# ArchieGertsman/spark-sched-sim

Hardware: AMD Instinct MI355X
Metric: env-steps/sec at 4096 batched envs (TPC-H, 10 exec) (higher is better)
Workload: dtype int64+f64

## Files before the change

### include/sss.h

```cpp
#ifndef SSS_H
#define SSS_H
#include <stddef.h>
#include <stdint.h>

#ifdef __cplusplus
extern "C" {
#endif

typedef struct sss_handle sss_handle;

typedef struct sss_cfg {
  int32_t num_executors;
  int32_t job_arrival_cap;
  int32_t max_jobs;
  int32_t reserved;
  double job_arrival_rate;
  double moving_delay;
  double warmup_delay;
  double beta;
} sss_cfg;

typedef struct sss_dims {
  int32_t num_envs, num_executors, job_cap, stage_stride;
  int32_t node_cap;
// ... 24 lines not shown
  SSS_E_STALLED = 5,
  SSS_E_NO_DURATION = 6,
  SSS_E_INVARIANT = 7,
  SSS_E_NEED_RESET = 8,
  SSS_E_NO_LIMIT = 9,
  SSS_E_CAPACITY = 10
};

int sss_query_dims(const sss_cfg* cfg, const void* pack, size_t pack_bytes, int num_envs, sss_dims* out);

int sss_create(const sss_cfg* cfg, const void* pack, size_t pack_bytes, int num_envs, int device, sss_handle** out);

int sss_bind_buffers(sss_handle* h, const sss_buffers* buffers);

int sss_reset(sss_handle* h, const uint64_t* seeds_dev, const double* time_limits_dev, const uint8_t* mask_dev, void* stream);

#define SSS_SKIP_ENV (-2147483647 - 1)
int sss_step(sss_handle* h, const int32_t* stage_idx_dev, const int32_t* num_exec_dev, int auto_reset, uint64_t seed_stride, void* stream);

int sss_step_bounded(sss_handle* h, const int32_t* stage_idx_dev, const int32_t* num_exec_dev, int auto_reset, uint64_t seed_stride, int max_events,
                     uint8_t* ready_dev, void* stream);

int sss_policy(sss_handle* h, int policy, int param, int32_t* stage_idx_dev, int32_t* num_exec_dev, void* stream);

int sss_rollout(sss_handle* h, int policy, int param, int n_steps, int auto_reset, uint64_t seed_stride, void* stream);

typedef struct sss_decima_graph {
  const uint8_t* active_dev;
  const int64_t* node_off_dev;
  const int64_t* job_off_dev;
  const int64_t* edge_off_dev;
  float num_tasks_scale;
  float work_scale;
  float* x_dev;
  int64_t* node_obs_dev;
  int64_t* node_loc_dev;
  int64_t* node_job_dev;
  int64_t* sched_rank_dev;
  int32_t* gen_dev;
  uint32_t* node_recv_dev;
  uint8_t* stage_mask_dev;
  int64_t* src_dev;
  int64_t* dst_dev;
  int64_t* edge_obs_dev;
  uint32_t* edge_layers_dev;
  int64_t* job_obs_dev;
// ... 383 lines not shown
```

### spark_sched_sim_amd/binding.py

```python
from __future__ import annotations

import ctypes as C
import os.path as osp

CSRC = osp.join(osp.dirname(osp.abspath(__file__)), "csrc")
LIB_NAME = "libsss_hip.so"


class SssCfg(C.Structure):
    _fields_ = [("num_executors", C.c_int32), ("job_arrival_cap", C.c_int32), ("max_jobs", C.c_int32),
                ("reserved", C.c_int32), ("job_arrival_rate", C.c_double), ("moving_delay", C.c_double),
                ("warmup_delay", C.c_double), ("beta", C.c_double)]


class SssDims(C.Structure):
    _fields_ = [("num_envs", C.c_int32), ("num_executors", C.c_int32), ("job_cap", C.c_int32),
                ("stage_stride", C.c_int32), ("node_cap", C.c_int32), ("edge_cap", C.c_int32),
                ("obs_i32", C.c_int32), ("obs_f64", C.c_int32), ("state_bytes", C.c_int64),
                ("env_stride", C.c_int64), ("off_t_arrival", C.c_int64), ("off_t_completed", C.c_int64),
                ("off_jobs", C.c_int64), ("off_active", C.c_int64), ("off_dur_ring", C.c_int64),
                ("job_rec_bytes", C.c_int32), ("hdr_bytes", C.c_int32)]


class SssBuffers(C.Structure):
# ... 137 lines not shown
    _fields_ = [("env_ids_dev", C.c_void_p), ("n", C.c_int32), ("width", C.c_int32), ("height", C.c_int32), ("pad_", C.c_int32), ("rgb_dev", C.c_void_p)]


JOB_STATS_COLUMNS = ("num_jobs", "total_job_time", "avg_job_duration", "avg_num_jobs", "avg_completed_job_duration", "num_completed_jobs", "num_active_jobs",
                     "wall_time")
JOB_STATS_MAX_Q = 16

REWARD_WINDOW_CHUNK = 64


def reward_window_scratch(T: int, B: int) -> int:
    return ((T + REWARD_WINDOW_CHUNK - 1) // REWARD_WINDOW_CHUNK + 1) * B + 1


class SssArenaArray(C.Structure):
    _fields_ = [("src_dev", C.c_void_p), ("dst_dev", C.c_void_p), ("elem_bytes", C.c_int32), ("per_row", C.c_int32), ("kind", C.c_int32), ("shift", C.c_int32)]


class SssArenaArgs(C.Structure):
    _fields_ = [("n_arrays", C.c_int32), ("n_obs", C.c_int32), ("totals_dev", C.c_void_p), ("cursor_dev", C.c_void_p), ("capacity", C.c_int64 * 4),
                ("rows_hint", C.c_int64), ("arrays", SssArenaArray * 24)]


EXPORTS = ["sss_query_dims", "sss_create", "sss_bind_buffers", "sss_reset", "sss_step", "sss_step_bounded", "sss_policy", "sss_rollout",
           "sss_decima_graph_build", "sss_decima_layer_lists", "sss_prefix_rows", "sss_decima_policy", "sss_decima_sample", "sss_gnn_launch",
           "sss_linear_wgrad_scratch", "sss_linear_wgrad", "sss_mlp_supported", "sss_mlp_recompute_supported", "sss_mlp_split_supported", "sss_mlp_forward", "sss_mlp_backward", "sss_mlp_wgrad_scratch", "sss_mlp_backward_wgrad", "sss_mlp_wgrad_finish", "sss_collect_step", "sss_gnn_encode", "sss_rows_op", "sss_rows_concat", "sss_segment_categorical", "sss_bit_lists", "sss_arena_append", "sss_discounted_returns", "sss_sequence_baselines", "sss_reward_window_update", "sss_differential_returns", "sss_bind_timeline", "sss_timeline_render", "sss_decima_argmax", "sss_decima_policy_argmax", "sss_job_stats", "sss_last_error", "sss_destroy", "sss_abi_sizeof"]
POLICY_IDS = {"fair": 0, "fifo": 1, "hash": 2, "wfair": 3, "sjfcp": 4}
WFAIR_ALPHA_RANGE = (-4, 4)
ABI_STRUCTS = {"sss_cfg": SssCfg, "sss_dims": SssDims, "sss_buffers": SssBuffers, "sss_decima_graph": SssDecimaGraph, "sss_decima_lists": SssDecimaLists,
               "sss_bit_list_args": SssBitListArgs, "sss_gnn_args": SssGnnArgs, "sss_decima_policy_args": SssDecimaPolicyArgs,
               "sss_decima_sample_args": SssDecimaSampleArgs, "sss_gnn_encode_args": SssGnnEncodeArgs, "sss_collect_args": SssCollectArgs,
               "sss_mlp_args": SssMlpArgs, "sss_arena_array": SssArenaArray, "sss_arena_args": SssArenaArgs, "sss_returns_args": SssReturnsArgs,
               "sss_baseline_args": SssBaselineArgs, "sss_rows_args": SssRowsArgs, "sss_concat_part": SssConcatPart, "sss_concat_args": SssConcatArgs, "sss_segcat_args": SssSegcatArgs}
ABI_TAGGED_STRUCTS = {"sss_reward_window_args": SssRewardWindowArgs, "sss_diffret_args": SssDiffretArgs}
ABI_PLAIN_STRUCTS = {"sss_timeline": SssTimeline, "sss_timeline_render_args": SssTimelineRenderArgs}


def load_library(path: str | None = None) -> C.CDLL:
    path = path or osp.join(CSRC, LIB_NAME)
    if not osp.exists(path):
        raise RuntimeError(
            f"{path} not found: the HIP extension has not been built "
            "(run `python -c 'import __graft_entry__ as g; g.build()'` or spark_sched_sim_amd/build.py). "
            "There is no CPU fallback.")
    return C.CDLL(path)


class Binding:
    def __init__(self, lib: C.CDLL | None = None):
        self.lib = lib if lib is not None else load_library()
        L = self.lib
        L.sss_query_dims.argtypes = [C.POINTER(SssCfg), C.c_void_p, C.c_size_t, C.c_int, C.POINTER(SssDims)]
        L.sss_create.argtypes = [C.POINTER(SssCfg), C.c_void_p, C.c_size_t, C.c_int, C.c_int, C.POINTER(C.c_void_p)]
        L.sss_bind_buffers.argtypes = [C.c_void_p, C.POINTER(SssBuffers)]
        L.sss_reset.argtypes = [C.c_void_p, C.c_void_p, C.c_void_p, C.c_void_p, C.c_void_p]
        L.sss_step.argtypes = [C.c_void_p, C.c_void_p, C.c_void_p, C.c_int, C.c_uint64, C.c_void_p]
        L.sss_step_bounded.argtypes = [C.c_void_p, C.c_void_p, C.c_void_p, C.c_int, C.c_uint64, C.c_int, C.c_void_p, C.c_void_p]
        L.sss_policy.argtypes = [C.c_void_p, C.c_int, C.c_int, C.c_void_p, C.c_void_p, C.c_void_p]
        L.sss_rollout.argtypes = [C.c_void_p, C.c_int, C.c_int, C.c_int, C.c_int, C.c_uint64, C.c_void_p]
        L.sss_decima_graph_build.argtypes = [C.c_void_p, C.POINTER(SssDecimaGraph), C.c_void_p]
        L.sss_decima_layer_lists.argtypes = [C.c_int, C.POINTER(SssDecimaLists), C.c_void_p]
        L.sss_prefix_rows.argtypes = [C.c_void_p, C.c_int64, C.c_int64, C.c_void_p, C.c_int, C.c_int, C.c_void_p, C.c_void_p, C.c_void_p, C.c_void_p]
        L.sss_decima_policy.argtypes = [C.c_void_p, C.POINTER(SssDecimaPolicyArgs), C.c_void_p]
        L.sss_decima_sample.argtypes = [C.c_int, C.c_int, C.POINTER(SssDecimaSampleArgs), C.c_void_p]
        L.sss_gnn_launch.argtypes = [C.c_int, C.POINTER(SssGnnArgs), C.c_void_p]
        L.sss_linear_wgrad_scratch.argtypes = [C.c_int, C.c_int]
        L.sss_linear_wgrad_scratch.restype = C.c_int64
        L.sss_linear_wgrad.argtypes = [C.c_void_p, C.c_int64, C.c_void_p, C.c_int64, C.c_int64, C.c_int, C.c_int, C.c_void_p, C.c_void_p, C.c_void_p, C.c_void_p]
        L.sss_gnn_encode.argtypes = [C.POINTER(SssGnnEncodeArgs), C.c_void_p]
        L.sss_collect_step.argtypes = [C.POINTER(SssCollectArgs), C.c_int, C.c_void_p]
        L.sss_mlp_supported.argtypes = [C.c_int] * 5
        L.sss_mlp_recompute_supported.argtypes = [C.c_int]
        L.sss_mlp_split_supported.argtypes = [C.c_int]
        L.sss_mlp_forward.argtypes = [C.POINTER(SssMlpArgs), C.c_void_p]
        L.sss_mlp_backward.argtypes = [C.POINTER(SssMlpArgs), C.c_void_p]
        L.sss_mlp_wgrad_scratch.argtypes = [C.c_int]
        L.sss_mlp_wgrad_scratch.restype = C.c_int64
        L.sss_mlp_backward_wgrad.argtypes = [C.POINTER(SssMlpArgs), C.c_void_p, C.c_void_p]
        L.sss_mlp_wgrad_finish.argtypes = [C.c_int] + [C.c_void_p] * 8
        L.sss_discounted_returns.argtypes = [C.POINTER(SssReturnsArgs), C.c_void_p]
# ... 46 lines not shown
```

### spark_sched_sim_amd/csrc/sss_hip_sim.hip

```cpp
#include <hip/hip_runtime.h>

#include "sss_sim.h"
#include "sss_narrow.h"

#ifdef SSS_TIMELINE
#define SSS_LAUNCHER(name) sss_narrow_tl_launch_##name
#define SSS_TL_DISPATCH(call)
#else
#define SSS_LAUNCHER(name) sss_narrow_launch_##name
#define SSS_TL_DISPATCH(call) \
  if (a.tl.t) return sss_narrow_tl_launch_##call
int sss_narrow_hot_bytes() { return (int)sizeof(SssHot); }
int sss_narrow_static_lds_bytes() { return SSS_STATIC_LDS_BYTES; }
#endif

int SSS_LAUNCHER(reset)(const SssKernelArgs& a, int num_envs, const uint64_t* seeds, const double* tl, const uint8_t* mask, void* stream) {
  SSS_TL_DISPATCH(reset(a, num_envs, seeds, tl, mask, stream));
  hipLaunchKernelGGL(SSS_KNAME(sss_reset_kernel), dim3(num_envs), dim3(64), (size_t)a.P.pool_bytes, (hipStream_t)stream, a, seeds, tl, mask);
  return (int)hipGetLastError();
}
int SSS_LAUNCHER(step_bounded)(const SssKernelArgs& a, int num_envs, const int32_t* stage_idx, const int32_t* num_exec, int auto_reset, uint64_t seed_stride,
                                   int budget, uint8_t* ready, void* stream) {
  SSS_TL_DISPATCH(step_bounded(a, num_envs, stage_idx, num_exec, auto_reset, seed_stride, budget, ready, stream));
  hipLaunchKernelGGL(SSS_KNAME(sss_step_bounded_kernel), dim3(num_envs), dim3(64), (size_t)a.P.pool_bytes, (hipStream_t)stream, a, stage_idx, num_exec, auto_reset, seed_stride,
                     budget, ready);
  return (int)hipGetLastError();
}
int SSS_LAUNCHER(step)(const SssKernelArgs& a, int num_envs, const int32_t* stage_idx, const int32_t* num_exec, int auto_reset, uint64_t seed_stride,
                           void* stream) {
  SSS_TL_DISPATCH(step(a, num_envs, stage_idx, num_exec, auto_reset, seed_stride, stream));
  hipLaunchKernelGGL(SSS_KNAME(sss_step_kernel), dim3(num_envs), dim3(64), (size_t)a.P.pool_bytes, (hipStream_t)stream, a, stage_idx, num_exec, auto_reset, seed_stride);
  return (int)hipGetLastError();
}
#ifndef SSS_TIMELINE
int SSS_LAUNCHER(policy)(const SssKernelArgs& a, int num_envs, int policy, int param, int32_t* stage_idx, int32_t* num_exec, void* stream) {
  hipLaunchKernelGGL(SSS_KNAME(sss_policy_kernel), dim3(num_envs), dim3(64), (size_t)a.P.pool_bytes, (hipStream_t)stream, a, policy, param, stage_idx, num_exec);
  return (int)hipGetLastError();
}
#endif
int SSS_LAUNCHER(rollout)(const SssKernelArgs& a, int num_envs, int policy, int param, int n_steps, int auto_reset, uint64_t seed_stride, void* stream) {
  SSS_TL_DISPATCH(rollout(a, num_envs, policy, param, n_steps, auto_reset, seed_stride, stream));
  if (policy >= SSS_POLICY_WFAIR)
    hipLaunchKernelGGL(SSS_KNAME(sss_rollout_heur_kernel), dim3(num_envs), dim3(64), (size_t)a.P.pool_bytes, (hipStream_t)stream, a, policy, param, n_steps, auto_reset, seed_stride);
  else
    hipLaunchKernelGGL(SSS_KNAME(sss_rollout_kernel), dim3(num_envs), dim3(64), (size_t)a.P.pool_bytes, (hipStream_t)stream, a, policy, param, n_steps, auto_reset, seed_stride);
  return (int)hipGetLastError();
}

#if defined(SSS_EVPROF3) && !defined(SSS_TIMELINE)
extern "C" int sss_debug_prof(unsigned long long* out64) {
  if (hipMemcpyFromSymbol(out64, HIP_SYMBOL(g_prof3), sizeof(unsigned long long) * 96) != hipSuccess) return -1;
  static const unsigned long long zeros[96] = {0};
  return hipMemcpyToSymbol(HIP_SYMBOL(g_prof3), zeros, sizeof(zeros)) == hipSuccess ? 0 : -1;
}
extern "C" int sss_debug_prof_min(unsigned long long min_step_ticks) {
  return hipMemcpyToSymbol(HIP_SYMBOL(g_prof3_min), &min_step_ticks, sizeof(min_step_ticks)) == hipSuccess ? 0 : -1;
}
#endif
```

### spark_sched_sim_amd/csrc/sss_hip_wide.hip

```cpp
#define SSS_WIDE 1
#include <hip/hip_runtime.h>

#include "sss_sim.h"
#include "sss_wide.h"

#ifdef SSS_TIMELINE
#define SSS_LAUNCHER(name) sss_wide_tl_launch_##name
#define SSS_TL_DISPATCH(call)
#else
#define SSS_LAUNCHER(name) sss_wide_launch_##name
#define SSS_TL_DISPATCH(call) \
  if (a.tl.t) return sss_wide_tl_launch_##call
int sss_wide_hot_bytes() { return (int)sizeof(SssHot); }
int sss_wide_static_lds_bytes() { return SSS_STATIC_LDS_BYTES; }
#endif

int SSS_LAUNCHER(reset)(const SssKernelArgs& a, int num_envs, const uint64_t* seeds, const double* tl, const uint8_t* mask, void* stream) {
  SSS_TL_DISPATCH(reset(a, num_envs, seeds, tl, mask, stream));
  hipLaunchKernelGGL(SSS_KNAME(sss_reset_kernel), dim3(num_envs), dim3(64), (size_t)a.P.pool_bytes, (hipStream_t)stream, a, seeds, tl, mask);
  return (int)hipGetLastError();
}
int SSS_LAUNCHER(step_bounded)(const SssKernelArgs& a, int num_envs, const int32_t* stage_idx, const int32_t* num_exec, int auto_reset, uint64_t seed_stride,
                                 int budget, uint8_t* ready, void* stream) {
  SSS_TL_DISPATCH(step_bounded(a, num_envs, stage_idx, num_exec, auto_reset, seed_stride, budget, ready, stream));
  hipLaunchKernelGGL(SSS_KNAME(sss_step_bounded_kernel), dim3(num_envs), dim3(64), (size_t)a.P.pool_bytes, (hipStream_t)stream, a, stage_idx, num_exec, auto_reset,
                     seed_stride, budget, ready);
  return (int)hipGetLastError();
}
int SSS_LAUNCHER(step)(const SssKernelArgs& a, int num_envs, const int32_t* stage_idx, const int32_t* num_exec, int auto_reset, uint64_t seed_stride,
                         void* stream) {
  SSS_TL_DISPATCH(step(a, num_envs, stage_idx, num_exec, auto_reset, seed_stride, stream));
  hipLaunchKernelGGL(SSS_KNAME(sss_step_kernel), dim3(num_envs), dim3(64), (size_t)a.P.pool_bytes, (hipStream_t)stream, a, stage_idx, num_exec, auto_reset, seed_stride);
  return (int)hipGetLastError();
}
#ifndef SSS_TIMELINE
int SSS_LAUNCHER(policy)(const SssKernelArgs& a, int num_envs, int policy, int param, int32_t* stage_idx, int32_t* num_exec, void* stream) {
  hipLaunchKernelGGL(SSS_KNAME(sss_policy_kernel), dim3(num_envs), dim3(64), (size_t)a.P.pool_bytes, (hipStream_t)stream, a, policy, param, stage_idx, num_exec);
  return (int)hipGetLastError();
}
#endif
int SSS_LAUNCHER(rollout)(const SssKernelArgs& a, int num_envs, int policy, int param, int n_steps, int auto_reset, uint64_t seed_stride, void* stream) {
  SSS_TL_DISPATCH(rollout(a, num_envs, policy, param, n_steps, auto_reset, seed_stride, stream));
  if (policy >= SSS_POLICY_WFAIR)
    hipLaunchKernelGGL(SSS_KNAME(sss_rollout_heur_kernel), dim3(num_envs), dim3(64), (size_t)a.P.pool_bytes, (hipStream_t)stream, a, policy, param, n_steps, auto_reset, seed_stride);
  else
    hipLaunchKernelGGL(SSS_KNAME(sss_rollout_kernel), dim3(num_envs), dim3(64), (size_t)a.P.pool_bytes, (hipStream_t)stream, a, policy, param, n_steps, auto_reset, seed_stride);
  return (int)hipGetLastError();
}

#if defined(SSS_EVPROF3) && !defined(SSS_TIMELINE)
extern "C" int sss_debug_prof_wide(unsigned long long* out64) {
  if (hipMemcpyFromSymbol(out64, HIP_SYMBOL(g_prof3), sizeof(unsigned long long) * 96) != hipSuccess) return -1;
  static const unsigned long long zeros[96] = {0};
  return hipMemcpyToSymbol(HIP_SYMBOL(g_prof3), zeros, sizeof(zeros)) == hipSuccess ? 0 : -1;
}
extern "C" int sss_debug_prof_min_wide(unsigned long long min_step_ticks) {
  return hipMemcpyToSymbol(HIP_SYMBOL(g_prof3_min), &min_step_ticks, sizeof(min_step_ticks)) == hipSuccess ? 0 : -1;
}
#endif
```

### spark_sched_sim_amd/csrc/sss_host.h

```cpp
#pragma once
#include <math.h>
#include <stdio.h>
#include <stdlib.h>
#include <string.h>

#include <string>
#include <vector>

#include "../../include/sss.h"
#include "sss_layout.h"
#include "sss_train.h"
#include "sss_rows.h"
#include "sss_narrow.h"
#include "sss_wide.h"
#include "sss_timeline.h"
#include "sss_jobstats.h"

static bool sss_is_wide(int num_executors) { return num_executors > 64; }
static int sss_hot_bytes(int num_executors) { return sss_is_wide(num_executors) ? sss_wide_hot_bytes() : sss_narrow_hot_bytes(); }

static thread_local std::string g_sss_err;
static int sss_fail(int code, const std::string& msg) {
  g_sss_err = msg;
  return code;
// ... 460 lines not shown
  if (max_events < 1) return sss_fail(-35, "sss_step_bounded: max_events must be at least 1");
  BeDeviceGuard guard(h->device);
  const SssKernelArgs ka = sss_args(h);
  if (int rc = sss_is_wide(h->L.E) ? sss_wide_launch_step_bounded(ka, h->L.num_envs, stage_idx_dev, num_exec_dev, auto_reset, seed_stride, max_events, ready_dev, stream)
                                   : be_launch_step_bounded(ka, h->L.num_envs, stage_idx_dev, num_exec_dev, auto_reset, seed_stride, max_events, ready_dev, stream))
    return sss_fail(-30, std::string("step launch failed: ") + be_error(rc));
  return 0;
}

static int sss_check_policy(int policy, int param) {
  if (policy < 0 || policy > 4) return sss_fail(-23, "unknown policy");
  if (policy == 3 && (param < -4 || param > 4)) return sss_fail(-23, "weighted fair: alpha (param) must be in [-4, 4], got " + std::to_string(param));
  return 0;
}

extern "C" int sss_policy(sss_handle* h, int policy, int param, int32_t* stage_idx_dev, int32_t* num_exec_dev, void* stream) {
  if (!h || !stage_idx_dev || !num_exec_dev) return sss_fail(-1, "NULL argument");
  if (!h->bound) return sss_fail(-22, "sss_bind_buffers has not been called");
  BeDeviceGuard guard(h->device);
  if (int rc = sss_check_policy(policy, param)) return rc;
  const SssKernelArgs ka = sss_args(h);
  if (int rc = sss_is_wide(h->L.E) ? sss_wide_launch_policy(ka, h->L.num_envs, policy, param, stage_idx_dev, num_exec_dev, stream)
                                   : be_launch_policy(ka, h->L.num_envs, policy, param, stage_idx_dev, num_exec_dev, stream)) return sss_fail(-30, std::string("policy launch failed: ") + be_error(rc));
  return 0;
}

extern "C" int sss_rollout(sss_handle* h, int policy, int param, int n_steps, int auto_reset, uint64_t seed_stride, void* stream) {
  if (!h) return sss_fail(-1, "NULL argument");
  if (!h->bound) return sss_fail(-22, "sss_bind_buffers has not been called");
  BeDeviceGuard guard(h->device);
  if (int rc = sss_check_policy(policy, param)) return rc;
  if (n_steps < 0) return sss_fail(-24, "n_steps must be >= 0");
  const SssKernelArgs ka = sss_args(h);
  if (int rc = sss_is_wide(h->L.E) ? sss_wide_launch_rollout(ka, h->L.num_envs, policy, param, n_steps, auto_reset, seed_stride, stream)
                                   : be_launch_rollout(ka, h->L.num_envs, policy, param, n_steps, auto_reset, seed_stride, stream)) return sss_fail(-30, std::string("rollout launch failed: ") + be_error(rc));
  return 0;
}

extern "C" int sss_decima_graph_build(sss_handle* h, const sss_decima_graph* g, void* stream) {
  if (!h || !g) return sss_fail(-1, "NULL argument");
  if (!h->bound) return sss_fail(-22, "sss_bind_buffers has not been called");
  BeDeviceGuard guard(h->device);
  if (!g->node_off_dev || !g->job_off_dev || !g->edge_off_dev || !g->x_dev || !g->node_obs_dev || !g->node_loc_dev || !g->node_job_dev ||
      !g->sched_rank_dev || !g->gen_dev || !g->node_recv_dev || !g->stage_mask_dev || !g->src_dev || !g->dst_dev || !g->edge_obs_dev ||
      !g->edge_layers_dev || !g->job_obs_dev || !g->job_cap_dev || !g->job_first_dev || !g->obs_depth_dev ||
      !g->job_nodes_dev || !g->out_start_dev || !g->out_deg_dev || !g->layer_cnt_dev)
// ... 471 lines not shown
```

### spark_sched_sim_amd/csrc/sss_narrow.h

```cpp
#pragma once
#include <stdint.h>

#include "sss_layout.h"

int sss_narrow_hot_bytes();
int sss_narrow_static_lds_bytes();
int sss_narrow_launch_reset(const SssKernelArgs& a, int num_envs, const uint64_t* seeds, const double* tl, const uint8_t* mask, void* stream);
int sss_narrow_launch_step_bounded(const SssKernelArgs& a, int num_envs, const int32_t* stage_idx, const int32_t* num_exec, int auto_reset, uint64_t seed_stride,
                                   int budget, uint8_t* ready, void* stream);
int sss_narrow_launch_step(const SssKernelArgs& a, int num_envs, const int32_t* stage_idx, const int32_t* num_exec, int auto_reset, uint64_t seed_stride, void* stream);
int sss_narrow_launch_policy(const SssKernelArgs& a, int num_envs, int policy, int param, int32_t* stage_idx, int32_t* num_exec, void* stream);
int sss_narrow_launch_rollout(const SssKernelArgs& a, int num_envs, int policy, int param, int n_steps, int auto_reset, uint64_t seed_stride, void* stream);
int sss_narrow_tl_launch_reset(const SssKernelArgs& a, int num_envs, const uint64_t* seeds, const double* tl, const uint8_t* mask, void* stream);
int sss_narrow_tl_launch_step_bounded(const SssKernelArgs& a, int num_envs, const int32_t* stage_idx, const int32_t* num_exec, int auto_reset, uint64_t seed_stride,
                                   int budget, uint8_t* ready, void* stream);
int sss_narrow_tl_launch_step(const SssKernelArgs& a, int num_envs, const int32_t* stage_idx, const int32_t* num_exec, int auto_reset, uint64_t seed_stride, void* stream);
int sss_narrow_tl_launch_rollout(const SssKernelArgs& a, int num_envs, int policy, int param, int n_steps, int auto_reset, uint64_t seed_stride, void* stream);
```

### spark_sched_sim_amd/csrc/sss_sim.h

```cpp
#pragma once
#ifdef SSS_WIDE
#ifdef SSS_TIMELINE
#define SSS_KNAME(name) name##_wide_tl
#else
#define SSS_KNAME(name) name##_wide
#endif
#else
#ifdef SSS_TIMELINE
#define SSS_KNAME(name) name##_tl
#else
#define SSS_KNAME(name) name
#endif
#endif
#include "../../include/sss.h"
#include "sss_layout.h"
#include <wave_rt.h>


struct alignas(16) SssScratch {
  uint8_t pool8[8];
  uint8_t pool8b[8];
  uint64_t rng_buf[64];
  int32_t rng_pos, pad0_[3];
  uint8_t setA[SSS_SET_TABLE];
// ... 269 lines not shown
#include "sss_sim_tracker.h"
#include "sss_sim_jobs.h"
#include "sss_sim_fulfil.h"
#include "sss_sim_events.h"
#include "sss_sim_fast_run.h"
#include "sss_sim_batches.h"
#include "sss_sim_lean.h"
#include "sss_sim_observe.h"
#include "sss_sim_env.h"
#undef SSS_SRC_ID
#define SSS_SRC_ID 0

SSS_KERNEL void SSS_KNAME(sss_reset_kernel)(SssKernelArgs a, const uint64_t* seeds, const double* time_limits, const uint8_t* mask) {
  int env = wave_env();
  if (mask && !mask[env]) return;
  uint8_t* base = (uint8_t*)a.B.state + (size_t)env * a.L.env_stride;
  ctx_init();
  env_begin(base);
  do_reset(a.L, seeds[env], time_limits ? time_limits[env] : __builtin_inf());
  write_observation(a.L, a.B, env, 0.0);
  env_end(base);
}

SSS_DEV void step_env(const SssKernelArgs& a, const int32_t* stage_idx, const int32_t* num_exec, int auto_reset, uint64_t seed_stride, int budget, uint8_t* ready) {
  int env = wave_env();
  if (stage_idx[env] == SSS_SKIP_ENV) return;
  uint8_t* base = (uint8_t*)a.B.state + (size_t)env * a.L.env_stride;
  ctx_init();
  env_begin(base);
  double reward = 0.0;
  bool yielded = false;
  bool start_next_episode = wave_ballot(auto_reset && g_hot.h.terminated && !g_hot.h.err) != 0;
  if (start_next_episode) {
    do_reset(a.L, g_hot.h.seed + seed_stride, g_hot.h.time_limit);
  } else {
    reward = do_step(stage_idx[env], num_exec[env], budget, &yielded);
  }
  if (!yielded) write_observation(a.L, a.B, env, reward);
  if (ready && wave_lane() == 0) ready[env] = yielded ? 0 : 1;
  env_end(base);
  prof3_flush();
}
SSS_KERNEL void SSS_KNAME(sss_step_kernel)(SssKernelArgs a, const int32_t* stage_idx, const int32_t* num_exec, int auto_reset, uint64_t seed_stride) {
  step_env(a, stage_idx, num_exec, auto_reset, seed_stride, 0, nullptr);
}
SSS_KERNEL void SSS_KNAME(sss_step_bounded_kernel)(SssKernelArgs a, const int32_t* stage_idx, const int32_t* num_exec, int auto_reset, uint64_t seed_stride,
                                                   int budget, uint8_t* ready) {
  step_env(a, stage_idx, num_exec, auto_reset, seed_stride, budget, ready);
}


SSS_DEV int obs_num_committable() {
  uint32_t srck = g_hot.h.curr_source;
  if (srck == POOL_NONE) return 0;
  int p = pool_index(srck);
  return (int)g_c.pool_hdr[p].used - (int)g_c.pool_hdr[p].commit_from;
}

SSS_DEV int find_stage_dev(uint64_t sm, uint64_t act, int gs) {
  int best = -1;
  uint64_t m = sm;
  while (m) {
// ... 208 lines not shown
  x += 0x9E3779B97F4A7C15ull;
  uint64_t z = x;
  z = (z ^ (z >> 30)) * 0xBF58476D1CE4E5B9ull;
  z = (z ^ (z >> 27)) * 0x94D049BB133111EBull;
  return z ^ (z >> 31);
}

SSS_DEV void policy_hash(int p_none_permille, int& stage_idx, int& num_exec) {
  uint64_t seed = g_hot.h.seed;
  uint64_t step = (uint64_t)g_hot.h.ep_steps;
  int n_sched = g_hot.h.n_sched;
  int ncommit = obs_num_committable();
  wave_sync();
  uint64_t h = splitmix64((seed << 32) ^ step), h2 = splitmix64(h), h3 = splitmix64(h2);
  if (n_sched == 0 || (int)(h3 % 1000) < p_none_permille)
    stage_idx = -1;
  else
    stage_idx = (int)(h % (uint64_t)n_sched);
  num_exec = 1 + (int)(h2 % (uint64_t)(ncommit > 0 ? ncommit : 1));
}

enum { SSS_POLICY_FAIR = 0, SSS_POLICY_FIFO = 1, SSS_POLICY_HASH = 2, SSS_POLICY_WFAIR = 3, SSS_POLICY_SJFCP = 4 };

template <bool kHeuristics = true>
SSS_DEV void run_policy(int policy, int param, int& stage_idx, int& num_exec) {
  PROF3(29);
  if (policy == SSS_POLICY_HASH)
    policy_hash(param, stage_idx, num_exec);
  else if (kHeuristics && policy == SSS_POLICY_WFAIR)
    policy_wfair(param, stage_idx, num_exec);
  else if (kHeuristics && policy == SSS_POLICY_SJFCP)
    policy_sjfcp(stage_idx, num_exec);
  else
    policy_fair(policy == SSS_POLICY_FAIR, stage_idx, num_exec);
}

#ifndef SSS_TIMELINE
SSS_KERNEL void SSS_KNAME(sss_policy_kernel)(SssKernelArgs a, int policy, int param, int32_t* stage_idx, int32_t* num_exec) {
  int env = wave_env();
  uint8_t* base = (uint8_t*)a.B.state + (size_t)env * a.L.env_stride;
  ctx_init();
  env_begin_readonly(base);
  int si, ne;
  run_policy(policy, param, si, ne);
  if (wave_lane() == 0) stage_idx[env] = si, num_exec[env] = ne;
}
#endif

#define ROLLOUT_BODY(kHeuristics) \
  int env = wave_env(); \
  uint8_t* base = (uint8_t*)a.B.state + (size_t)env * a.L.env_stride; \
  ctx_init(); \
  env_begin(base); \
  for (int it = 0; it < n_steps; it++) { \
    bool over = wave_ballot(g_hot.h.terminated || g_hot.h.need_reset) != 0; \
    double reward = 0.0; \
    if (over) { \
      if (!auto_reset || wave_ballot(g_hot.h.err != 0) != 0) break;  \
      do_reset(a.L, g_hot.h.seed + seed_stride, g_hot.h.time_limit); \
    } else { \
      int si, ne; \
      run_policy<kHeuristics>(policy, param, si, ne); \
      reward = do_step<true>(si, ne); \
    } \
    write_observation(a.L, a.B, env, reward); \
    wave_sync(); \
  } \
  env_end(base); \
  prof3_flush();
// ... 21 lines not shown
```

### spark_sched_sim_amd/csrc/sss_wide.h

```cpp
#pragma once
#include <stdint.h>

#include "sss_layout.h"

int sss_wide_hot_bytes();
int sss_wide_static_lds_bytes();
int sss_wide_launch_reset(const SssKernelArgs& a, int num_envs, const uint64_t* seeds, const double* tl, const uint8_t* mask, void* stream);
int sss_wide_launch_step_bounded(const SssKernelArgs& a, int num_envs, const int32_t* stage_idx, const int32_t* num_exec, int auto_reset, uint64_t seed_stride,
                                 int budget, uint8_t* ready, void* stream);
int sss_wide_launch_step(const SssKernelArgs& a, int num_envs, const int32_t* stage_idx, const int32_t* num_exec, int auto_reset, uint64_t seed_stride, void* stream);
int sss_wide_launch_policy(const SssKernelArgs& a, int num_envs, int policy, int param, int32_t* stage_idx, int32_t* num_exec, void* stream);
int sss_wide_launch_rollout(const SssKernelArgs& a, int num_envs, int policy, int param, int n_steps, int auto_reset, uint64_t seed_stride, void* stream);
int sss_wide_tl_launch_reset(const SssKernelArgs& a, int num_envs, const uint64_t* seeds, const double* tl, const uint8_t* mask, void* stream);
int sss_wide_tl_launch_step_bounded(const SssKernelArgs& a, int num_envs, const int32_t* stage_idx, const int32_t* num_exec, int auto_reset, uint64_t seed_stride,
                                 int budget, uint8_t* ready, void* stream);
int sss_wide_tl_launch_step(const SssKernelArgs& a, int num_envs, const int32_t* stage_idx, const int32_t* num_exec, int auto_reset, uint64_t seed_stride, void* stream);
int sss_wide_tl_launch_rollout(const SssKernelArgs& a, int num_envs, int policy, int param, int n_steps, int auto_reset, uint64_t seed_stride, void* stream);
```

### spark_sched_sim_amd/vec_env.py

```python
from __future__ import annotations

import ctypes as C
from typing import Any, Sequence

import numpy as np
import torch

from . import workload
from .binding import (ERROR_NAMES, POLICY_IDS, WFAIR_ALPHA_RANGE, Binding, SssBuffers, SssCfg, SssDecimaGraph, SssDecimaLists, SssTimeline,
                      SssTimelineRenderArgs, device_of)

OBS_FIELDS = ("n_nodes", "n_edges", "n_jobs", "n_schedulable", "num_committable_execs", "source_job_idx",
              "terminated", "err")
NUM_NODE_FEATURES = 3


class BatchedObs(dict):
    """dict of device tensors; rows beyond n_nodes[i] / n_edges[i] / n_jobs[i] of env i are padding.

    keys: nodes f32[B, node_cap, 3], edge_links i32[B, edge_cap, 2], dag_ptr i32[B, job_cap+1],
    exec_supplies i32[B, job_cap], plus one i32[B] tensor per OBS_FIELDS entry.
    """


# ... 22 lines not shown

    def read_tagged(self):
        for k in (self.last, 1 - self.last):
            if self.posted[k] and (not self.cuda or self.events[k].query()):
                self.kept = (self.bufs[k].clone(), self.tags[k])
                break
        kept = getattr(self, "kept", None)
        return (kept[0].clone(), kept[1]) if kept is not None else (self.fill.clone(), None)

    def post(self, t: torch.Tensor, tag=None) -> None:
        k = 1 - self.last
        if self.cuda and self.posted[k] and not self.events[k].query():
            return
        self.bufs[k].copy_(t, non_blocking=True)
        if self.cuda:
            self.events[k].record(torch.cuda.current_stream(t.device))
        self.posted[k], self.last, self.tags[k] = True, k, tag


class VecSparkSchedSimEnv:

    def __init__(self, env_cfg: dict[str, Any], num_envs: int, device: str | torch.device = "cuda:0",
                 pack: bytes | None = None, auto_reset: bool = False, seed_stride: int | None = None,
                 _lib: C.CDLL | None = None) -> None:
        self.device = torch.device(device)
        if self.device.type != "cuda" and _lib is None:
            raise RuntimeError("VecSparkSchedSimEnv runs on an AMD GPU (device='cuda:N'); there is no CPU path")
        sampler = env_cfg.get("data_sampler_cls", "TPCHDataSampler")
        if sampler != "TPCHDataSampler":
            raise ValueError(f"'{sampler}' is not a valid data sampler.")
        self.num_envs = int(num_envs)
        self.num_executors = int(env_cfg["num_executors"])
        self.env_cfg = dict(env_cfg)
        self.auto_reset = bool(auto_reset)
        self.seed_stride = int(seed_stride if seed_stride is not None else num_envs)
        self._b = Binding(_lib)
        self._pack = pack if pack is not None else workload.default_pack()
        cap = env_cfg.get("job_arrival_cap")
        self._cfg = SssCfg(self.num_executors, int(cap) if cap else 0, int(env_cfg.get("max_jobs") or 0), 0,
                           float(env_cfg["job_arrival_rate"]), float(env_cfg["moving_delay"]),
                           float(env_cfg["warmup_delay"]), float(env_cfg.get("beta", 0.0)))
        self.dims = self._b.query_dims(self._cfg, self._pack, self.num_envs)
        dev_index = self.device.index or 0
        self._h = self._b.create(self._cfg, self._pack, self.num_envs, dev_index if self.device.type == "cuda" else -1)
        d, B, dev = self.dims, self.num_envs, self.device
        self._state_raw = torch.zeros(d.state_bytes + 256, dtype=torch.uint8, device=dev)
        off = (-self._state_raw.data_ptr()) % 256
        self.state = self._state_raw[off: off + d.state_bytes]
        self.nodes = torch.zeros((B, d.node_cap, NUM_NODE_FEATURES), dtype=torch.float32, device=dev)
        self.edge_links = torch.zeros((B, d.edge_cap, 2), dtype=torch.int32, device=dev)
        self.dag_ptr = torch.zeros((B, d.job_cap + 1), dtype=torch.int32, device=dev)
        self.exec_supplies = torch.zeros((B, d.job_cap), dtype=torch.int32, device=dev)
        self.obs_i32 = torch.zeros((B, d.obs_i32), dtype=torch.int32, device=dev)
        self.obs_f64 = torch.zeros((B, d.obs_f64), dtype=torch.float64, device=dev)
        self.rebind_buffers()
        self._seeds = torch.zeros(B, dtype=torch.int64, device=dev)
        self._tl = torch.full((B,), float("inf"), dtype=torch.float64, device=dev)
        self._mask = torch.ones(B, dtype=torch.uint8, device=dev)
        self._env_view = self.state.view(B, d.env_stride)
        self._act_stage = torch.zeros(B, dtype=torch.int32, device=dev)
        self._act_nexec = torch.ones(B, dtype=torch.int32, device=dev)
        self._closed = False
        self._dg_pool: dict[int, torch.Tensor] = {}
        self._layer_scratch: dict = {}
        self._never = None
        from .workload import pack_max_depth
        self.max_dag_depth = pack_max_depth(self._pack)
        from .spaces import make_action_space, make_observation_space
        self.single_action_space = make_action_space(self.num_executors)
        self.action_space = self.single_action_space
        self.single_observation_space = make_observation_space(self.num_executors, NUM_NODE_FEATURES)
        self.observation_space = self.single_observation_space


    def rebind_buffers(self) -> None:
        bufs = SssBuffers(self.state.data_ptr(), self.nodes.data_ptr(), self.edge_links.data_ptr(),
                          self.dag_ptr.data_ptr(), self.exec_supplies.data_ptr(), self.obs_i32.data_ptr(),
                          self.obs_f64.data_ptr())
        self._b.check(self._b.lib.sss_bind_buffers(self._h, C.byref(bufs)))
        self._bind_timeline()

    def _stream(self) -> int:
        return torch.cuda.current_stream(self.device).cuda_stream if self.device.type == "cuda" else 0

    def _obs(self) -> BatchedObs:
        o = BatchedObs(nodes=self.nodes, edge_links=self.edge_links, dag_ptr=self.dag_ptr,
                       exec_supplies=self.exec_supplies)
        for k, name in enumerate(OBS_FIELDS):
            o[name] = self.obs_i32[:, k]
        return o

    def close(self) -> None:
        if not self._closed:
            if self.device.type == "cuda":
                torch.cuda.synchronize(self.device)
            self._b.lib.sss_destroy(self._h)
            self._closed = True

    def __del__(self):
        try:
            self.close()
        except Exception:
            pass


    def reset(self, *, seed: int | Sequence[int] | None = None, options: dict[str, Any] | None = None,
              mask: torch.Tensor | None = None):
        B = self.num_envs
        if seed is None:
            seeds = np.random.SeedSequence().generate_state(B, np.uint64) >> np.uint64(1)
        elif isinstance(seed, (int, np.integer)):
            seeds = np.arange(B, dtype=np.uint64) + np.uint64(int(seed))
        else:
            seeds = np.asarray(list(seed), dtype=np.uint64)
            if seeds.shape != (B,):
                raise ValueError("need one seed per env")
        self._seeds.copy_(torch.from_numpy(seeds.view(np.int64)))
        tl = (options or {}).get("time_limit", np.inf)
        tl_arr = np.broadcast_to(np.asarray(tl, dtype=np.float64), (B,)).copy()
        self._tl.copy_(torch.from_numpy(tl_arr))
        mask_ptr = None
        if mask is not None:
            self._mask.copy_(mask.to(torch.uint8))
            mask_ptr = self._mask.data_ptr()
        self._b.check(self._b.lib.sss_reset(self._h, self._seeds.data_ptr(), self._tl.data_ptr(), mask_ptr, self._stream()))
        return self._obs(), {"wall_time": self.obs_f64[:, 1]}

    def step_async(self, stage_idx: torch.Tensor, num_exec: torch.Tensor) -> None:
        assert stage_idx.dtype == torch.int32 and num_exec.dtype == torch.int32
        assert stage_idx.device == self.device and stage_idx.is_contiguous() and num_exec.is_contiguous()
        self._b.check(self._b.lib.sss_step(self._h, stage_idx.data_ptr(), num_exec.data_ptr(), int(self.auto_reset),
                                           self.seed_stride, self._stream()))

    def step_bounded_async(self, stage_idx: torch.Tensor, num_exec: torch.Tensor, max_events: int, ready: torch.Tensor | None = None) -> torch.Tensor:
        assert stage_idx.dtype == torch.int32 and num_exec.dtype == torch.int32
        assert stage_idx.device == self.device and stage_idx.is_contiguous() and num_exec.is_contiguous()
        if ready is None:
            if getattr(self, "_ready", None) is None:
                self._ready = torch.ones(self.num_envs, dtype=torch.uint8, device=self.device)
            ready = self._ready
        assert ready.dtype == torch.uint8 and ready.is_contiguous() and ready.numel() == self.num_envs
        self._b.check(self._b.lib.sss_step_bounded(self._h, stage_idx.data_ptr(), num_exec.data_ptr(), int(self.auto_reset), self.seed_stride, int(max_events),
                                                   ready.data_ptr(), self._stream()))
        return ready

    def step(self, actions):
        if set(actions.keys()) != {"stage_idx", "num_exec"}:
            raise ValueError("invalid action: does not belong to the action space")
        self.step_async(actions["stage_idx"], actions["num_exec"])
        obs = self._obs()
        f64 = self.obs_f64.clone()
        i32 = self.obs_i32[:, 6:8].clone()
        terminated = i32[:, 0] != 0
        if self._never is None or self._never.shape != terminated.shape:
            self._never = torch.zeros_like(terminated)
        return obs, f64[:, 0], terminated, self._never, {"wall_time": f64[:, 1], "err": i32[:, 1]}


    def _bind_timeline(self) -> None:
        tl = getattr(self, "_timeline", None)
        if tl is None:
            self._b.check(self._b.lib.sss_bind_timeline(self._h, None))
            return
        t, job, count = tl
# ... 35 lines not shown
        dev = self.device
        if env_ids is None:
            ids, n = None, self.num_envs
        else:
            ids = torch.as_tensor(env_ids, dtype=torch.int32).reshape(-1).to(dev).contiguous()
            n = int(ids.numel())
            if n and (int(ids.min()) < 0 or int(ids.max()) >= self.num_envs):
                raise IndexError("render: env id out of range")
        rgb = torch.empty((n, int(height), int(width), 3), dtype=torch.uint8, device=dev)
        a = SssTimelineRenderArgs(ids.data_ptr() if ids is not None and n else None, n, int(width), int(height), 0, rgb.data_ptr() if n else None)
        self._b.check(self._b.lib.sss_timeline_render(self._h, C.byref(a), self._stream()))
        return rgb


    @staticmethod
    def _policy_id(policy: str, param: int) -> int:
        pid = POLICY_IDS[policy]
        lo, hi = WFAIR_ALPHA_RANGE
        if policy == "wfair" and not lo <= int(param) <= hi:
            raise ValueError(f"wfair: alpha (param) must be an integer in [{lo}, {hi}], got {param}")
        return pid

    def policy_actions(self, policy: str = "fair", param: int = 0):
        pid = self._policy_id(policy, param)
        self._b.check(self._b.lib.sss_policy(self._h, pid, int(param), self._act_stage.data_ptr(),
                                             self._act_nexec.data_ptr(), self._stream()))
        return {"stage_idx": self._act_stage, "num_exec": self._act_nexec}

    def rollout(self, policy: str, n_steps: int, param: int = 0) -> None:
        pid = self._policy_id(policy, param)
        self._b.check(self._b.lib.sss_rollout(self._h, pid, int(param), int(n_steps), int(self.auto_reset),
                                              self.seed_stride, self._stream()))

    def decima_graph_on_device(self, active: torch.Tensor | None = None, num_tasks_scale: float = 200.0, work_scale: float = 1e5) -> dict[str, Any]:
        B, dev, d = self.num_envs, self.device, self.dims
        assert self.graph_kernel_fits, "the graph kernel's LDS working set does not fit this node capacity"
        D = self.max_dag_depth
        ws = getattr(self, "_dg_dev", None)
        if ws is None:
            Mc, Ec, Jc = B * d.node_cap, B * d.edge_cap, B * d.job_cap
            e = lambda n, dt, *tail: torch.empty((max(n, 1), *tail), dtype=dt, device=dev)
            ws = self._dg_dev = {
                "x": e(Mc, torch.float32, 5), "node_obs": e(Mc, torch.int64), "node_loc": e(Mc, torch.int64), "node_job": e(Mc, torch.int64),
                "sched_rank": e(Mc, torch.int64), "gen": e(Mc, torch.int32), "node_recv": e(Mc, torch.int32), "stage_mask": e(Mc, torch.bool),
                "src": e(Ec, torch.int64), "dst": e(Ec, torch.int64), "edge_obs": e(Ec, torch.int64), "edge_layers": e(Ec, torch.int32),
                "job_obs": e(Jc, torch.int64), "job_cap": e(Jc, torch.int64), "job_first": e(Jc, torch.int64), "obs_depth": e(B, torch.int32),
                "job_nodes": e(Jc, torch.int64), "out_start": e(Mc, torch.int64), "out_deg": e(Mc, torch.int32),
                "layer_cnt": e(32, torch.int32, B), "sched_list": e(Mc, torch.int64),
                "scan": e(2, torch.int64, 4, B),
                "pp": torch.zeros(1056 + 4 + 1056, dtype=torch.int64, device=dev),
                "recv": e(Mc * max(D, 1), torch.int64), "hint": LateHint(1060, dev), "epoch": 0}
            ws["tot"] = ws["pp"][1056:1060]
        act8 = _mask_u8(active)
# ... 275 lines not shown
```

Before: 24.04 million.

## Fuse next-step heuristic policy into step kernel with double-buffered actions

Adds a step_prepare kernel that, after advancing each env, runs the heuristic policy in the same wave and writes the next action into spare buffers. The Python wrapper remembers the last requested policy, launches the fused kernel when the step uses its own action buffers, and on the next policy_actions call swaps buffers instead of launching the policy kernel. This removes one kernel launch and one reload of env state per step. The cost is generation bookkeeping to invalidate stale precomputed actions and extra work when the caller asks for a different policy.

```diff
diff --git a/include/sss.h b/include/sss.h
--- a/include/sss.h
+++ b/include/sss.h
@@ -70,6 +70,9 @@
                      uint8_t* ready_dev, void* stream);
 
 int sss_policy(sss_handle* h, int policy, int param, int32_t* stage_idx_dev, int32_t* num_exec_dev, void* stream);
+
+int sss_step_prepare(sss_handle* h, const int32_t* stage_idx_dev, const int32_t* num_exec_dev, int auto_reset, uint64_t seed_stride, int policy, int param,
+                     int32_t* next_stage_idx_dev, int32_t* next_num_exec_dev, void* stream);
 
 int sss_rollout(sss_handle* h, int policy, int param, int n_steps, int auto_reset, uint64_t seed_stride, void* stream);
 
diff --git a/spark_sched_sim_amd/binding.py b/spark_sched_sim_amd/binding.py
--- a/spark_sched_sim_amd/binding.py
+++ b/spark_sched_sim_amd/binding.py
@@ -183,7 +183,7 @@
                 ("rows_hint", C.c_int64), ("arrays", SssArenaArray * 24)]
 
 
-EXPORTS = ["sss_query_dims", "sss_create", "sss_bind_buffers", "sss_reset", "sss_step", "sss_step_bounded", "sss_policy", "sss_rollout",
+EXPORTS = ["sss_query_dims", "sss_create", "sss_bind_buffers", "sss_reset", "sss_step", "sss_step_bounded", "sss_step_prepare", "sss_policy", "sss_rollout",
            "sss_decima_graph_build", "sss_decima_layer_lists", "sss_prefix_rows", "sss_decima_policy", "sss_decima_sample", "sss_gnn_launch",
            "sss_linear_wgrad_scratch", "sss_linear_wgrad", "sss_mlp_supported", "sss_mlp_recompute_supported", "sss_mlp_split_supported", "sss_mlp_forward", "sss_mlp_backward", "sss_mlp_wgrad_scratch", "sss_mlp_backward_wgrad", "sss_mlp_wgrad_finish", "sss_collect_step", "sss_gnn_encode", "sss_rows_op", "sss_rows_concat", "sss_segment_categorical", "sss_bit_lists", "sss_arena_append", "sss_discounted_returns", "sss_sequence_baselines", "sss_reward_window_update", "sss_differential_returns", "sss_bind_timeline", "sss_timeline_render", "sss_decima_argmax", "sss_decima_policy_argmax", "sss_job_stats", "sss_last_error", "sss_destroy", "sss_abi_sizeof"]
 POLICY_IDS = {"fair": 0, "fifo": 1, "hash": 2, "wfair": 3, "sjfcp": 4}
@@ -217,6 +217,7 @@
         L.sss_reset.argtypes = [C.c_void_p, C.c_void_p, C.c_void_p, C.c_void_p, C.c_void_p]
         L.sss_step.argtypes = [C.c_void_p, C.c_void_p, C.c_void_p, C.c_int, C.c_uint64, C.c_void_p]
         L.sss_step_bounded.argtypes = [C.c_void_p, C.c_void_p, C.c_void_p, C.c_int, C.c_uint64, C.c_int, C.c_void_p, C.c_void_p]
+        L.sss_step_prepare.argtypes = [C.c_void_p, C.c_void_p, C.c_void_p, C.c_int, C.c_uint64, C.c_int, C.c_int, C.c_void_p, C.c_void_p, C.c_void_p]
         L.sss_policy.argtypes = [C.c_void_p, C.c_int, C.c_int, C.c_void_p, C.c_void_p, C.c_void_p]
         L.sss_rollout.argtypes = [C.c_void_p, C.c_int, C.c_int, C.c_int, C.c_int, C.c_uint64, C.c_void_p]
         L.sss_decima_graph_build.argtypes = [C.c_void_p, C.POINTER(SssDecimaGraph), C.c_void_p]
diff --git a/spark_sched_sim_amd/csrc/sss_hip_sim.hip b/spark_sched_sim_amd/csrc/sss_hip_sim.hip
--- a/spark_sched_sim_amd/csrc/sss_hip_sim.hip
+++ b/spark_sched_sim_amd/csrc/sss_hip_sim.hip
@@ -37,6 +37,12 @@
   hipLaunchKernelGGL(SSS_KNAME(sss_policy_kernel), dim3(num_envs), dim3(64), (size_t)a.P.pool_bytes, (hipStream_t)stream, a, policy, param, stage_idx, num_exec);
   return (int)hipGetLastError();
 }
+int SSS_LAUNCHER(step_prepare)(const SssKernelArgs& a, int num_envs, const int32_t* stage_idx, const int32_t* num_exec, int auto_reset, uint64_t seed_stride,
+                               int policy, int param, int32_t* next_stage, int32_t* next_nexec, void* stream) {
+  hipLaunchKernelGGL(SSS_KNAME(sss_step_prepare_kernel), dim3(num_envs), dim3(64), (size_t)a.P.pool_bytes, (hipStream_t)stream, a, stage_idx, num_exec, auto_reset,
+                     seed_stride, policy, param, next_stage, next_nexec);
+  return (int)hipGetLastError();
+}
 #endif
 int SSS_LAUNCHER(rollout)(const SssKernelArgs& a, int num_envs, int policy, int param, int n_steps, int auto_reset, uint64_t seed_stride, void* stream) {
   SSS_TL_DISPATCH(rollout(a, num_envs, policy, param, n_steps, auto_reset, seed_stride, stream));
diff --git a/spark_sched_sim_amd/csrc/sss_hip_wide.hip b/spark_sched_sim_amd/csrc/sss_hip_wide.hip
--- a/spark_sched_sim_amd/csrc/sss_hip_wide.hip
+++ b/spark_sched_sim_amd/csrc/sss_hip_wide.hip
@@ -38,6 +38,12 @@
   hipLaunchKernelGGL(SSS_KNAME(sss_policy_kernel), dim3(num_envs), dim3(64), (size_t)a.P.pool_bytes, (hipStream_t)stream, a, policy, param, stage_idx, num_exec);
   return (int)hipGetLastError();
 }
+int SSS_LAUNCHER(step_prepare)(const SssKernelArgs& a, int num_envs, const int32_t* stage_idx, const int32_t* num_exec, int auto_reset, uint64_t seed_stride,
+                               int policy, int param, int32_t* next_stage, int32_t* next_nexec, void* stream) {
+  hipLaunchKernelGGL(SSS_KNAME(sss_step_prepare_kernel), dim3(num_envs), dim3(64), (size_t)a.P.pool_bytes, (hipStream_t)stream, a, stage_idx, num_exec, auto_reset,
+                     seed_stride, policy, param, next_stage, next_nexec);
+  return (int)hipGetLastError();
+}
 #endif
 int SSS_LAUNCHER(rollout)(const SssKernelArgs& a, int num_envs, int policy, int param, int n_steps, int auto_reset, uint64_t seed_stride, void* stream) {
   SSS_TL_DISPATCH(rollout(a, num_envs, policy, param, n_steps, auto_reset, seed_stride, stream));
diff --git a/spark_sched_sim_amd/csrc/sss_host.h b/spark_sched_sim_amd/csrc/sss_host.h
--- a/spark_sched_sim_amd/csrc/sss_host.h
+++ b/spark_sched_sim_amd/csrc/sss_host.h
@@ -506,6 +506,21 @@
   const SssKernelArgs ka = sss_args(h);
   if (int rc = sss_is_wide(h->L.E) ? sss_wide_launch_policy(ka, h->L.num_envs, policy, param, stage_idx_dev, num_exec_dev, stream)
                                    : be_launch_policy(ka, h->L.num_envs, policy, param, stage_idx_dev, num_exec_dev, stream)) return sss_fail(-30, std::string("policy launch failed: ") + be_error(rc));
+  return 0;
+}
+
+extern "C" int sss_step_prepare(sss_handle* h, const int32_t* stage_idx_dev, const int32_t* num_exec_dev, int auto_reset, uint64_t seed_stride, int policy, int param,
+                                int32_t* next_stage_idx_dev, int32_t* next_num_exec_dev, void* stream) {
+  if (!h || !stage_idx_dev || !num_exec_dev || !next_stage_idx_dev || !next_num_exec_dev) return sss_fail(-1, "NULL argument");
+  if (!h->bound) return sss_fail(-22, "sss_bind_buffers has not been called");
+  if (h->tl.t) return sss_fail(-43, "sss_step_prepare: a timeline is bound - there is no recording form of this launch (use sss_step and sss_policy)");
+  if (stage_idx_dev == next_stage_idx_dev || num_exec_dev == next_num_exec_dev) return sss_fail(-43, "sss_step_prepare: the next action must go to buffers of its own");
+  BeDeviceGuard guard(h->device);
+  if (int rc = sss_check_policy(policy, param)) return rc;
+  const SssKernelArgs ka = sss_args(h);
+  if (int rc = sss_is_wide(h->L.E) ? sss_wide_launch_step_prepare(ka, h->L.num_envs, stage_idx_dev, num_exec_dev, auto_reset, seed_stride, policy, param, next_stage_idx_dev, next_num_exec_dev, stream)
+                                   : sss_narrow_launch_step_prepare(ka,h->L.num_envs, stage_idx_dev, num_exec_dev, auto_reset, seed_stride, policy, param, next_stage_idx_dev, next_num_exec_dev, stream))
+    return sss_fail(-30, std::string("step launch failed: ") + be_error(rc));
   return 0;
 }
 
diff --git a/spark_sched_sim_amd/csrc/sss_narrow.h b/spark_sched_sim_amd/csrc/sss_narrow.h
--- a/spark_sched_sim_amd/csrc/sss_narrow.h
+++ b/spark_sched_sim_amd/csrc/sss_narrow.h
@@ -10,6 +10,8 @@
                                    int budget, uint8_t* ready, void* stream);
 int sss_narrow_launch_step(const SssKernelArgs& a, int num_envs, const int32_t* stage_idx, const int32_t* num_exec, int auto_reset, uint64_t seed_stride, void* stream);
 int sss_narrow_launch_policy(const SssKernelArgs& a, int num_envs, int policy, int param, int32_t* stage_idx, int32_t* num_exec, void* stream);
+int sss_narrow_launch_step_prepare(const SssKernelArgs& a, int num_envs, const int32_t* stage_idx, const int32_t* num_exec, int auto_reset, uint64_t seed_stride,
+                                  int policy, int param, int32_t* next_stage, int32_t* next_nexec, void* stream);
 int sss_narrow_launch_rollout(const SssKernelArgs& a, int num_envs, int policy, int param, int n_steps, int auto_reset, uint64_t seed_stride, void* stream);
 int sss_narrow_tl_launch_reset(const SssKernelArgs& a, int num_envs, const uint64_t* seeds, const double* tl, const uint8_t* mask, void* stream);
 int sss_narrow_tl_launch_step_bounded(const SssKernelArgs& a, int num_envs, const int32_t* stage_idx, const int32_t* num_exec, int auto_reset, uint64_t seed_stride,
diff --git a/spark_sched_sim_amd/csrc/sss_sim.h b/spark_sched_sim_amd/csrc/sss_sim.h
--- a/spark_sched_sim_amd/csrc/sss_sim.h
+++ b/spark_sched_sim_amd/csrc/sss_sim.h
@@ -315,9 +315,21 @@
   env_end(base);
 }
 
-SSS_DEV void step_env(const SssKernelArgs& a, const int32_t* stage_idx, const int32_t* num_exec, int auto_reset, uint64_t seed_stride, int budget, uint8_t* ready) {
+template <bool kHeuristics = true> SSS_DEV void run_policy(int policy, int param, int& stage_idx, int& num_exec);
+template <bool kPrepare = false>
+SSS_DEV void step_env(const SssKernelArgs& a, const int32_t* stage_idx, const int32_t* num_exec, int auto_reset, uint64_t seed_stride, int budget, uint8_t* ready,
+                      int policy = 0, int param = 0, int32_t* next_stage = nullptr, int32_t* next_nexec = nullptr) {
   int env = wave_env();
-  if (stage_idx[env] == SSS_SKIP_ENV) return;
+  if (stage_idx[env] == SSS_SKIP_ENV) {
+    if (kPrepare) {
+      ctx_init();
+      env_begin_readonly((const uint8_t*)a.B.state + (size_t)env * a.L.env_stride);
+      int si, ne;
+      run_policy<true>(policy, param, si, ne);
+      if (wave_lane() == 0) next_stage[env] = si, next_nexec[env] = ne;
+    }
+    return;
+  }
   uint8_t* base = (uint8_t*)a.B.state + (size_t)env * a.L.env_stride;
   ctx_init();
   env_begin(base);
@@ -331,6 +343,12 @@
   }
   if (!yielded) write_observation(a.L, a.B, env, reward);
   if (ready && wave_lane() == 0) ready[env] = yielded ? 0 : 1;
+  if (kPrepare) {
+    wave_sync();
+    int si, ne;
+    run_policy<true>(policy, param, si, ne);
+    if (wave_lane() == 0) next_stage[env] = si, next_nexec[env] = ne;
+  }
   env_end(base);
   prof3_flush();
 }
@@ -585,7 +603,7 @@
 
 enum { SSS_POLICY_FAIR = 0, SSS_POLICY_FIFO = 1, SSS_POLICY_HASH = 2, SSS_POLICY_WFAIR = 3, SSS_POLICY_SJFCP = 4 };
 
-template <bool kHeuristics = true>
+template <bool kHeuristics>
 SSS_DEV void run_policy(int policy, int param, int& stage_idx, int& num_exec) {
   PROF3(29);
   if (policy == SSS_POLICY_HASH)
@@ -608,6 +626,30 @@
   run_policy(policy, param, si, ne);
   if (wave_lane() == 0) stage_idx[env] = si, num_exec[env] = ne;
 }
+#endif
+
+#ifndef SSS_TIMELINE
+SSS_KERNEL void SSS_KNAME(sss_step_prepare_kernel)(SssKernelArgs a, const int32_t* stage_idx, const int32_t* num_exec, int auto_reset, uint64_t seed_stride,
+                                                   int policy, int param, int32_t* next_stage, int32_t* next_nexec) {
+  step_env<true>(a, stage_idx, num_exec, auto_reset, seed_stride, 0, nullptr, policy, param, next_stage, next_nexec);
+}
+#ifndef __HIP__
+#include <functional>
+namespace emu {
+void launch(int grid, const std::function<void()>& body);
+}
+#ifdef SSS_WIDE
+int sss_wide_launch_step_prepare
+#else
+int sss_narrow_launch_step_prepare
+#endif
+    (const SssKernelArgs& a, int num_envs, const int32_t* stage_idx, const int32_t* num_exec, int auto_reset, uint64_t seed_stride, int policy, int param,
+     int32_t* next_stage, int32_t* next_nexec, void*) {
+  emu::g_kernargs = &a;
+  emu::launch(num_envs, [&]() { SSS_KNAME(sss_step_prepare_kernel)(a, stage_idx, num_exec, auto_reset, seed_stride, policy, param, next_stage, next_nexec); });
+  return 0;
+}
+#endif
 #endif
 
 #define ROLLOUT_BODY(kHeuristics) \
diff --git a/spark_sched_sim_amd/csrc/sss_wide.h b/spark_sched_sim_amd/csrc/sss_wide.h
--- a/spark_sched_sim_amd/csrc/sss_wide.h
+++ b/spark_sched_sim_amd/csrc/sss_wide.h
@@ -10,6 +10,8 @@
                                  int budget, uint8_t* ready, void* stream);
 int sss_wide_launch_step(const SssKernelArgs& a, int num_envs, const int32_t* stage_idx, const int32_t* num_exec, int auto_reset, uint64_t seed_stride, void* stream);
 int sss_wide_launch_policy(const SssKernelArgs& a, int num_envs, int policy, int param, int32_t* stage_idx, int32_t* num_exec, void* stream);
+int sss_wide_launch_step_prepare(const SssKernelArgs& a, int num_envs, const int32_t* stage_idx, const int32_t* num_exec, int auto_reset, uint64_t seed_stride,
+                                int policy, int param, int32_t* next_stage, int32_t* next_nexec, void* stream);
 int sss_wide_launch_rollout(const SssKernelArgs& a, int num_envs, int policy, int param, int n_steps, int auto_reset, uint64_t seed_stride, void* stream);
 int sss_wide_tl_launch_reset(const SssKernelArgs& a, int num_envs, const uint64_t* seeds, const double* tl, const uint8_t* mask, void* stream);
 int sss_wide_tl_launch_step_bounded(const SssKernelArgs& a, int num_envs, const int32_t* stage_idx, const int32_t* num_exec, int auto_reset, uint64_t seed_stride,
diff --git a/spark_sched_sim_amd/vec_env.py b/spark_sched_sim_amd/vec_env.py
--- a/spark_sched_sim_amd/vec_env.py
+++ b/spark_sched_sim_amd/vec_env.py
@@ -68,7 +68,7 @@
 
     def __init__(self, env_cfg: dict[str, Any], num_envs: int, device: str | torch.device = "cuda:0",
                  pack: bytes | None = None, auto_reset: bool = False, seed_stride: int | None = None,
-                 _lib: C.CDLL | None = None) -> None:
+                 _lib: C.CDLL | None = None, fuse_policy: bool = True) -> None:
         self.device = torch.device(device)
         if self.device.type != "cuda" and _lib is None:
             raise RuntimeError("VecSparkSchedSimEnv runs on an AMD GPU (device='cuda:N'); there is no CPU path")
@@ -80,6 +80,10 @@
         self.env_cfg = dict(env_cfg)
         self.auto_reset = bool(auto_reset)
         self.seed_stride = int(seed_stride if seed_stride is not None else num_envs)
+        self.fuse_policy = bool(fuse_policy)
+        self._gen = 0
+        self._asked = None
+        self._prepared = None
         self._b = Binding(_lib)
         self._pack = pack if pack is not None else workload.default_pack()
         cap = env_cfg.get("job_arrival_cap")
@@ -106,6 +110,7 @@
         self._env_view = self.state.view(B, d.env_stride)
         self._act_stage = torch.zeros(B, dtype=torch.int32, device=dev)
         self._act_nexec = torch.ones(B, dtype=torch.int32, device=dev)
+        self._act_spare = (torch.zeros(B, dtype=torch.int32, device=dev), torch.ones(B, dtype=torch.int32, device=dev))
         self._closed = False
         self._dg_pool: dict[int, torch.Tensor] = {}
         self._layer_scratch: dict = {}
@@ -120,11 +125,15 @@
 
 
     def rebind_buffers(self) -> None:
+        self._touch()
         bufs = SssBuffers(self.state.data_ptr(), self.nodes.data_ptr(), self.edge_links.data_ptr(),
                           self.dag_ptr.data_ptr(), self.exec_supplies.data_ptr(), self.obs_i32.data_ptr(),
                           self.obs_f64.data_ptr())
         self._b.check(self._b.lib.sss_bind_buffers(self._h, C.byref(bufs)))
         self._bind_timeline()
+
+    def _touch(self) -> None:
+        self._gen += 1
 
     def _stream(self) -> int:
         return torch.cuda.current_stream(self.device).cuda_stream if self.device.type == "cuda" else 0
@@ -137,6 +146,7 @@
         return o
 
     def close(self) -> None:
+        self._touch()
         if not self._closed:
             if self.device.type == "cuda":
                 torch.cuda.synchronize(self.device)
@@ -169,14 +179,24 @@
         if mask is not None:
             self._mask.copy_(mask.to(torch.uint8))
             mask_ptr = self._mask.data_ptr()
+        self._touch()
         self._b.check(self._b.lib.sss_reset(self._h, self._seeds.data_ptr(), self._tl.data_ptr(), mask_ptr, self._stream()))
         return self._obs(), {"wall_time": self.obs_f64[:, 1]}
 
     def step_async(self, stage_idx: torch.Tensor, num_exec: torch.Tensor) -> None:
         assert stage_idx.dtype == torch.int32 and num_exec.dtype == torch.int32
         assert stage_idx.device == self.device and stage_idx.is_contiguous() and num_exec.is_contiguous()
-        self._b.check(self._b.lib.sss_step(self._h, stage_idx.data_ptr(), num_exec.data_ptr(), int(self.auto_reset),
-                                           self.seed_stride, self._stream()))
+        self._touch()
+        sp, np_, stream = stage_idx.data_ptr(), num_exec.data_ptr(), self._stream()
+        asked = self._asked
+        if (self.fuse_policy and asked is not None and sp == self._act_stage.data_ptr() and np_ == self._act_nexec.data_ptr()
+                and getattr(self, "_timeline", None) is None):
+            nxt_stage, nxt_nexec = self._act_spare
+            self._b.check(self._b.lib.sss_step_prepare(self._h, sp, np_, int(self.auto_reset), self.seed_stride, asked[0], asked[1],
+                                                       nxt_stage.data_ptr(), nxt_nexec.data_ptr(), stream))
+            self._prepared = (asked[0], asked[1], stream, self._gen)
+            return
+        self._b.check(self._b.lib.sss_step(self._h, sp, np_, int(self.auto_reset), self.seed_stride, stream))
 
     def step_bounded_async(self, stage_idx: torch.Tensor, num_exec: torch.Tensor, max_events: int, ready: torch.Tensor | None = None) -> torch.Tensor:
         assert stage_idx.dtype == torch.int32 and num_exec.dtype == torch.int32
@@ -186,6 +206,7 @@
                 self._ready = torch.ones(self.num_envs, dtype=torch.uint8, device=self.device)
             ready = self._ready
         assert ready.dtype == torch.uint8 and ready.is_contiguous() and ready.numel() == self.num_envs
+        self._touch()
         self._b.check(self._b.lib.sss_step_bounded(self._h, stage_idx.data_ptr(), num_exec.data_ptr(), int(self.auto_reset), self.seed_stride, int(max_events),
                                                    ready.data_ptr(), self._stream()))
         return ready
@@ -267,13 +288,20 @@
         return pid
 
     def policy_actions(self, policy: str = "fair", param: int = 0):
-        pid = self._policy_id(policy, param)
-        self._b.check(self._b.lib.sss_policy(self._h, pid, int(param), self._act_stage.data_ptr(),
-                                             self._act_nexec.data_ptr(), self._stream()))
+        pid, param, stream = self._policy_id(policy, param), int(param), self._stream()
+        self._asked = (pid, param)
+        if self._prepared == (pid, param, stream, self._gen):
+            spare = self._act_spare
+            self._act_spare = (self._act_stage, self._act_nexec)
+            self._act_stage, self._act_nexec = spare
+            self._prepared = None
+        else:
+            self._b.check(self._b.lib.sss_policy(self._h, pid, param, self._act_stage.data_ptr(), self._act_nexec.data_ptr(), stream))
         return {"stage_idx": self._act_stage, "num_exec": self._act_nexec}
 
     def rollout(self, policy: str, n_steps: int, param: int = 0) -> None:
         pid = self._policy_id(policy, param)
+        self._touch()
         self._b.check(self._b.lib.sss_rollout(self._h, pid, int(param), int(n_steps), int(self.auto_reset),
                                               self.seed_stride, self._stream()))
 
```

Result: no change. 24.24 million, median of 6 (+0.8%).
